# Sujit-O/pykg2vec

Hardware: AMD Instinct MI355X
Metric: scored triples/sec (train) + test-triples ranked/sec, FB15k TransE d=100 (higher is better)
Workload: dtype f32

## Files before the change

pykg2vec_amd/csrc/kge_eval.hip:

```cpp
#include "kge_internal.h"
#include <stdlib.h>
#include <string.h>

namespace kge {

#ifndef KGE_GEMM_CHUNK
#define KGE_GEMM_CHUNK 64
#endif
constexpr int kGemmChunk = KGE_GEMM_CHUNK;
constexpr int KC = 8;
constexpr int QT_PLAIN = 16;
constexpr int QT_XF = 8;

enum Form { F_L1 = 0, F_L2 = 1, F_SQM = 2, F_NEGDOT = 3 };
enum XForm { X_NONE = 0, X_TRANSH = 1, X_TRANSD = 2 };
enum Post { P_NONE = 0, P_SCALE = 1, P_CLAMP = 2, P_SIGMOID = 3 };

struct EvalPlan {
    int64_t nq;
    int only;
    int64_t E, n, tables, table_stride;
    int K, Kpad, QV, form, xform, post;
    int64_t ntiles;
    float* cand; float* aux; float* qvec; float* qscale; float* st; int32_t* fcount; int32_t* rcount; int32_t* tcount;
    float* qT;
    size_t bytes;
};

static int sweep_K(const kge_model_desc* m) {
    switch (m->model) {
        case KGE_COMPLEX: case KGE_ROTATE: case KGE_ANALOGY: return 2 * m->dim;
        case KGE_CP: case KGE_SIMPLE: case KGE_SIMPLE_IGNR: return 2 * m->dim;
        case KGE_QUATE: return 4 * m->dim;
        case KGE_TRANSR: return m->rel_dim;
        case KGE_HEAD_1N_INTERNAL: return m->dim + (m->tables[1] ? 1 : 0);
        default: return m->dim;
    }
}

static bool make_plan(const kge_model_desc* m, int64_t n, void* ws, EvalPlan* p, int64_t tables = 1) {
    p->E = m->tot_entity; p->n = n; p->nq = 2 * n; p->only = 2; p->tables = tables;
    const bool per_group_tables = tables > 1 || m->model == KGE_TRANSR;
    p->K = sweep_K(m);
    p->Kpad = (p->K + KC - 1) / KC * KC;
    p->xform = per_group_tables ? X_NONE : m->model == KGE_TRANSH ? X_TRANSH : m->model == KGE_TRANSD ? X_TRANSD : X_NONE;
    p->QV = p->xform == X_NONE ? 1 : 2;
    switch (m->model) {
        case KGE_TRANSE: case KGE_TRANSH: case KGE_TRANSD: case KGE_TRANSM: case KGE_TRANSR:
            p->form = (m->flags & KGE_FLAG_L1) ? F_L1 : F_L2; break;
        case KGE_ROTATE: p->form = F_SQM; break;
        case KGE_DISTMULT: case KGE_COMPLEX: case KGE_ANALOGY: case KGE_RESCAL:
        case KGE_CP: case KGE_SIMPLE: case KGE_SIMPLE_IGNR: case KGE_QUATE: case KGE_HEAD_1N_INTERNAL: case KGE_DOT_INTERNAL: p->form = F_NEGDOT; break;
        default: return false;
    }
    p->post = m->model == KGE_TRANSM ? P_SCALE : (m->model == KGE_SIMPLE || m->model == KGE_SIMPLE_IGNR) ? P_CLAMP
              : (m->model == KGE_HEAD_1N_INTERNAL || (m->model == KGE_DOT_INTERNAL && (m->flags & kDotSigmoid))) ? P_SIGMOID : P_NONE;
    p->ntiles = (p->E + 63) / 64;
    const bool dot_form = (p->form == F_NEGDOT || p->form == F_SQM) && p->xform == X_NONE;
    if (dot_form) p->Kpad = (p->K + 15) / 16 * 16;
    size_t off = 0;
    char* base = (char*)ws;
    auto take = [&](size_t bytes) { char* q = base ? base + off : nullptr; off += align256(bytes); return q; };
    p->table_stride = p->ntiles * p->Kpad * 64;
    p->cand = (float*)take(((size_t)tables * p->table_stride + (dot_form ? (size_t)p->Kpad * 64 : 0)) * sizeof(float));
    p->aux = (float*)take((size_t)p->ntiles * 64 * sizeof(float));
    p->qvec = (float*)take((size_t)2 * n * p->QV * p->Kpad * sizeof(float));
    p->qscale = (float*)take((size_t)2 * n * sizeof(float));
    p->st = (float*)take((size_t)2 * n * sizeof(float));
    p->fcount = (int32_t*)take((size_t)2 * n * sizeof(int32_t));
    p->rcount = (int32_t*)take((size_t)4 * n * sizeof(int32_t));
    p->tcount = p->rcount ? p->rcount + 2 * n : nullptr;
    p->qT = nullptr;
    if ((p->form == F_NEGDOT || p->form == F_SQM) && p->xform == X_NONE)
        p->qT = (float*)take((size_t)((2 * n + 127) / 128) * p->Kpad * 128 * sizeof(float));
    p->bytes = off;
    return true;
}

size_t eval_workspace_bytes(const kge_model_desc* m, int64_t n, int64_t tables) {
    if (WsBytesFn* own = model_ops(m->model)->eval_ws) return own(m, n);
    EvalPlan p;
    if (!make_plan(m, n, nullptr, &p, tables)) return 0;
    return p.bytes;
}

// ... 357 lines not shown
        for (int k = lane; k < dc; k += TPT) {
            qt[base + k] = hr[k] * rr[k] - hi[k] * ri[k];
            qt[base + dc + k] = hi[k] * rr[k] + hr[k] * ri[k];
            qh[base + k] = tr[k] * rr[k] + ti[k] * ri[k];
            qh[base + dc + k] = ti[k] * rr[k] - tr[k] * ri[k];
        }
        if constexpr (M == KGE_ANALOGY) {
            const float* eh = m.tab[0] + h * d; const float* er = m.tab[1] + r * d; const float* et = m.tab[0] + t * d;
            for (int k = lane; k < d; k += TPT) { qt[k] = eh[k] * er[k]; qh[k] = er[k] * et[k]; }
        }
    } else if constexpr (M == KGE_ROTATE) {
        const float* hr = m.tab[0] + h * d; const float* hi = m.tab[1] + h * d; const float* rl = m.tab[2] + r * d;
        const float* tr = m.tab[0] + t * d; const float* ti = m.tab[1] + t * d;
        for (int k = lane; k < d; k += TPT) {
            float sn, cs;
            sincosf(rl[k] / m.phase_div, &sn, &cs);
            qt[k] = hr[k] * cs - hi[k] * sn;
            qt[d + k] = hr[k] * sn + hi[k] * cs;
            qh[k] = tr[k] * cs + ti[k] * sn;
            qh[d + k] = ti[k] * cs - tr[k] * sn;
        }
    } else if constexpr (M == KGE_CP) {
        const float* sh = m.tab[0] + h * d; const float* er = m.tab[1] + r * d; const float* ot = m.tab[2] + t * d;
        for (int k = lane; k < d; k += TPT) {
            qt[k] = 0.f; qt[d + k] = sh[k] * er[k];
            qh[k] = er[k] * ot[k]; qh[d + k] = 0.f;
        }
    } else if constexpr (M == KGE_SIMPLE || M == KGE_SIMPLE_IGNR) {
        const float w2 = (M == KGE_SIMPLE) ? 0.5f : 1.0f;
        const float* hh = m.tab[0] + h * d; const float* ht = m.tab[0] + t * d;
        const float* th = m.tab[1] + h * d; const float* tt = m.tab[1] + t * d;
        const float* r1 = m.tab[2] + r * d; const float* r2 = m.tab[3] + r * d;
        for (int k = lane; k < d; k += TPT) {
            qt[k] = hh[k] * r1[k];
            qt[d + k] = w2 * (r2[k] * th[k]);
            qh[k] = w2 * (ht[k] * r2[k]);
            qh[d + k] = r1[k] * tt[k];
        }
    } else if constexpr (M == KGE_QUATE) {
        const float* H[4]; const float* T[4]; const float* Rq[4];
        for (int c = 0; c < 4; ++c) { H[c] = m.tab[c] + h * d; T[c] = m.tab[c] + t * d; Rq[c] = m.tab[4 + c] + r * d; }
        for (int k = lane; k < d; k += TPT) {
            const float rs = Rq[0][k], rx = Rq[1][k], ry = Rq[2][k], rz = Rq[3][k];
            const float den = sqrtf(rs * rs + rx * rx + ry * ry + rz * rz);
            const float inv = den > 0.f ? 1.0f / den : 0.f;
            const float ps = rs * inv, px = rx * inv, py = ry * inv, pz = rz * inv;
            const float hs = H[0][k], hx = H[1][k], hy = H[2][k], hz = H[3][k];
            const float ts = T[0][k], tx = T[1][k], ty = T[2][k], tz = T[3][k];
            qt[k] = hs * ps - hx * px - hy * py - hz * pz;
            qt[d + k] = hs * px + ps * hx + hy * pz - py * hz;
            qt[2 * d + k] = hs * py + ps * hy + hz * px - pz * hx;
            qt[3 * d + k] = hs * pz + ps * hz + hx * py - px * hy;
            qh[k] = ps * ts + px * tx + py * ty + pz * tz;
            qh[d + k] = -px * ts + ps * tx - pz * ty + py * tz;
            qh[2 * d + k] = -py * ts + pz * tx + ps * ty - px * tz;
            qh[3 * d + k] = -pz * ts - py * tx + px * ty + ps * tz;
        }
    } else if constexpr (M == KGE_RESCAL) {
        const float* eh = m.tab[0] + h * d; const float* et = m.tab[0] + t * d;
        const float* Mr = m.tab[1] + r * (int64_t)d * d;
        for (int j = lane; j < d; j += TPT) {
            float a = 0.f, b = 0.f;
            int i2 = 0;
            for (; i2 + KC <= d; i2 += KC) {
                float m1[KC], m2[KC], hv[KC], tv[KC];
#pragma unroll
                for (int u = 0; u < KC; ++u) {
                    m1[u] = Mr[(int64_t)(i2 + u) * d + j]; m2[u] = Mr[(int64_t)j * d + i2 + u];
                    hv[u] = eh[i2 + u]; tv[u] = et[i2 + u];
                }
#pragma unroll
                for (int u = 0; u < KC; ++u) { a = fmaf(hv[u], m1[u], a); b = fmaf(m2[u], tv[u], b); }
            }
            for (; i2 < d; ++i2) {
                a = fmaf(eh[i2], Mr[(int64_t)i2 * d + j], a);
                b = fmaf(Mr[(int64_t)j * d + i2], et[i2], b);
            }
            qt[j] = a; qh[j] = b;
        }
    }
}

__device__ __forceinline__ float add_abs(float acc, float d) { return acc + fabsf(d); }

__device__ __forceinline__ float fma_sq(float acc, float d) {
    float r;
    asm("v_fma_f32 %0, %1, %1, %2" : "=v"(r) : "v"(d), "v"(acc));
    return r;
}

template <int FORM>
__device__ __forceinline__ float pair_step(float acc, float c, float q) {
    if constexpr (FORM == F_L1) return add_abs(acc, c - q);
    else if constexpr (FORM == F_NEGDOT) return fmaf(c, q, acc);
    else { const float dlt = c - q; return fma_sq(acc, dlt); }
}
template <int FORM>
__device__ __forceinline__ float pair_finish(float acc, float margin) {
    if constexpr (FORM == F_L1) return acc;
    else if constexpr (FORM == F_L2) return sqrtf(acc);
    else if constexpr (FORM == F_SQM) return -(margin - acc);
    else return -acc;
}

template <int POST>
__device__ __forceinline__ float pair_post(float s, float scale) {
    if constexpr (POST == P_SCALE) return scale * s;
    else if constexpr (POST == P_CLAMP) return fminf(fmaxf(s, -20.f), 20.f);
    else if constexpr (POST == P_SIGMOID) return -(1.0f / (1.0f + expf(s)));
    else return s;
}

__device__ __forceinline__ float sqm_from_dot(float dot, float qn, float cn) { return fmaf(-2.0f, dot, qn + cn); }

template <int FORM, int XFORM, int POST>
__device__ __forceinline__ float pair_score_lane(const float* __restrict__ cand, const float* __restrict__ aux,
                                                 const float* __restrict__ q, int64_t e, int Kpad, float margin,
                                                 float scale) {
    const float* c = cand + ((e >> 6) * Kpad) * 64 + (e & 63);
    float acc = 0.f;
    if constexpr (XFORM == X_NONE && FORM != F_L1) {
        float a0 = 0.f, a1 = 0.f;
        for (int k0 = 0; k0 < Kpad; k0 += KC) {
            float cv[KC], qv[KC];
#pragma unroll
            for (int j = 0; j < KC; ++j) { cv[j] = c[(int64_t)(k0 + j) * 64]; qv[j] = q[k0 + j]; }
#pragma unroll
            for (int j = 0; j < KC; j += 2) {
                if constexpr (FORM == F_NEGDOT) {
                    a0 = fmaf(cv[j], qv[j], a0);
                    a1 = fmaf(cv[j + 1], qv[j + 1], a1);
                } else {
                    const float d0 = cv[j] - qv[j], d1 = cv[j + 1] - qv[j + 1];
                    a0 = fmaf(d0, d0, a0);
                    a1 = fmaf(d1, d1, a1);
                }
            }
        }
        acc = a0 + a1;
    } else if constexpr (XFORM == X_NONE) {
        constexpr int KL = 32;
        int k0 = 0;
        for (; k0 + KL <= Kpad; k0 += KL) {
            float cv[KL], qv[KL];
#pragma unroll
            for (int j = 0; j < KL; ++j) { cv[j] = c[(int64_t)(k0 + j) * 64]; qv[j] = q[k0 + j]; }
#pragma unroll
            for (int j = 0; j < KL; ++j) acc = pair_step<FORM>(acc, cv[j], qv[j]);
        }
        for (; k0 < Kpad; k0 += KC) {
            float cv[KC], qv[KC];
#pragma unroll
            for (int j = 0; j < KC; ++j) { cv[j] = c[(int64_t)(k0 + j) * 64]; qv[j] = q[k0 + j]; }
#pragma unroll
            for (int j = 0; j < KC; ++j) acc = pair_step<FORM>(acc, cv[j], qv[j]);
        }
    } else {
        const float* w = q + Kpad;
        float p;
        if constexpr (XFORM == X_TRANSH) {
            p = 0.f;
            for (int k0 = 0; k0 < Kpad; k0 += KC) {
                float cv[KC], wv[KC];
#pragma unroll
                for (int j = 0; j < KC; ++j) { cv[j] = c[(int64_t)(k0 + j) * 64]; wv[j] = w[k0 + j]; }
#pragma unroll
// ... 113 lines not shown
                    const int kk = k0 + (t & (ch - 1));
                    int ee = lc_u >= 6 ? __builtin_amdgcn_readlane(e, (64 * u) >> lc_u) : __shfl(e, (t >> lc_u) & 63, 64);
                    asm volatile("" : "+v"(ee));
                    const float* src = prep_addr(a, ee, kk);
                    if (t < total && src) v[u] = *src;
                }
            }
#pragma unroll
            for (int u = 0; u < 4; ++u) {
                const int kk = 64 * u + lane;
                qv[u] = (kk < ch && k0 + kk < Kpad) ? q[k0 + kk] : 0.f;
            }
        };
        fetch(0);
        for (int k0 = 0; k0 < Kpad; k0 += ch) {
#pragma unroll
            for (int u = 0; u < 16; ++u) {
                const int t = 64 * u + lane;
                if (64 * u < total_u && t < total) sc[(t >> lc) * pitch + (t & (ch - 1))] = v[u];
            }
#pragma unroll
            for (int u = 0; u < 4; ++u) {
                const int kk = 64 * u + lane;
                if (kk < ch) sq[kk] = qv[u];
            }
            if (k0 + ch < Kpad) fetch(k0 + ch);
            __builtin_amdgcn_wave_barrier();
            __builtin_amdgcn_s_waitcnt(0xC07F);
            if (lane < pg) {
                const float* cr = sc + lane * pitch;
                const int nk = min(ch, Kpad - k0);
                int kk = 0;
                for (; kk + 16 <= nk; kk += 16) {
                    float4 c4[4], q4[4];
#pragma unroll
                    for (int u = 0; u < 4; ++u) {
                        c4[u] = *reinterpret_cast<const float4*>(cr + kk + 4 * u);
                        q4[u] = *reinterpret_cast<const float4*>(sq + kk + 4 * u);
                    }
#pragma unroll
                    for (int u = 0; u < 4; ++u) {
                        acc = fmaf(c4[u].x, q4[u].x, acc); acc = fmaf(c4[u].y, q4[u].y, acc);
                        acc = fmaf(c4[u].z, q4[u].z, acc); acc = fmaf(c4[u].w, q4[u].w, acc);
                    }
                    if (kGemmChunk && ((k0 + kk + 16) % (kGemmChunk ? kGemmChunk : 1)) == 0) { tot += acc; acc = 0.f; }
                }
                for (; kk < nk; kk += 8) {
                    const float4 c0 = *reinterpret_cast<const float4*>(cr + kk), c1 = *reinterpret_cast<const float4*>(cr + kk + 4);
                    const float4 q0 = *reinterpret_cast<const float4*>(sq + kk), q1 = *reinterpret_cast<const float4*>(sq + kk + 4);
                    acc = fmaf(c0.x, q0.x, acc); acc = fmaf(c0.y, q0.y, acc); acc = fmaf(c0.z, q0.z, acc); acc = fmaf(c0.w, q0.w, acc);
                    acc = fmaf(c1.x, q1.x, acc); acc = fmaf(c1.y, q1.y, acc); acc = fmaf(c1.z, q1.z, acc); acc = fmaf(c1.w, q1.w, acc);
                    if (kGemmChunk && ((k0 + kk + 8) % (kGemmChunk ? kGemmChunk : 1)) == 0) { tot += acc; acc = 0.f; }
                }
            }
            __builtin_amdgcn_wave_barrier();
        }
        if (kGemmChunk) acc = tot + acc;
        if constexpr (FORM == F_SQM) acc = sqm_from_dot(acc, qn, lane < pg ? aux[e] : 0.f);
        const float sco = pair_post<POST>(pair_finish<FORM>(acc, margin), 1.0f);
        if (base == 0) s_true = __shfl(sco, 0, 64);
        if (lane < pg && idx > 0 && e != truth) cnt += (sco < s_true) ? 1 : 0;
        base += pg;
    }
    cnt = (int)wave_sum((float)cnt);
    if (lane == 0) { st[qi] = s_true; fcount[qi] = cnt; }
}

typedef float f32x2 __attribute__((ext_vector_type(2)));

template <int FORM>
__device__ __forceinline__ void pair_step2(float& acc, f32x2 c, f32x2 q) {
    if constexpr (FORM == F_NEGDOT) {
        acc = fmaf(c.x, q.x, acc);
        acc = fmaf(c.y, q.y, acc);
    } else if constexpr (FORM == F_L1) {
        acc = add_abs(acc, c.x - q.x);
        acc = add_abs(acc, c.y - q.y);
    } else {
        const f32x2 d = c - q;
        acc = fma_sq(acc, d.x); acc = fma_sq(acc, d.y);
    }
}

template <int QT, int NS, class F>
__device__ __forceinline__ void for_query_chunks(const float* const (&qrow)[QT], const int (&off)[NS], F body) {
    float nx[NS][KC];
#pragma unroll
    for (int s = 0; s < NS; ++s)
#pragma unroll
        for (int j = 0; j < KC; ++j) nx[s][j] = qrow[0][off[s] + j];
#pragma unroll
    for (int q = 0; q < QT; ++q) {
        float cur[NS][KC];
#pragma unroll
        for (int s = 0; s < NS; ++s)
#pragma unroll
            for (int j = 0; j < KC; ++j) cur[s][j] = nx[s][j];
#pragma unroll
        for (int s = 0; s < NS; ++s) asm volatile("" ::"s"(cur[s][0]), "s"(cur[s][KC - 1]));
        if (q + 1 < QT) {
#pragma unroll
            for (int s = 0; s < NS; ++s)
#pragma unroll
                for (int j = 0; j < KC; ++j) nx[s][j] = qrow[q + 1][off[s] + j];
        }
        __builtin_amdgcn_sched_barrier(0);
        body(q, cur);
        __builtin_amdgcn_sched_barrier(0);
    }
}

template <int FORM, int XFORM, int QT, bool WRITE, int POST>
__global__ __launch_bounds__(256) void k_eval_sweep(const float* __restrict__ cand, const float* __restrict__ aux,
                                                    const float* __restrict__ qvec, const float* __restrict__ qscale,
                                                    const float* __restrict__ st,
                                                    int64_t nq, int64_t E, int64_t ntiles, int Kpad, int QV, float margin,
                                                    int S, int qblocks, int32_t* __restrict__ rcount,
                                                    int32_t* __restrict__ tcount, float* __restrict__ scores_out,
                                                    const int32_t* __restrict__ qdesc, int64_t table_stride) {
    const int lane = threadIdx.x & 63;
    const int wave = threadIdx.x >> 6;
    const int slot = blockIdx.x & 255;
    const int mm = blockIdx.x >> 8;
    const int ts = mm % S;
    const int qb = (mm / S) * 256 + slot;
    if (qb >= qblocks) return;
    int64_t q0 = (int64_t)qb * QT;
    if (qdesc) {
        cand += qdesc[4 * qb] * table_stride;
        q0 = qdesc[4 * qb + 1];
        nq = q0 + qdesc[4 * qb + 2];
    }
    const int64_t qstride = (int64_t)QV * Kpad;
    const float* qrow[QT];
    float sthr[QT];
    float qsc[QT];
    int cnt[QT];
    int tie[QT];
#pragma unroll
    for (int q = 0; q < QT; ++q) {
        const int64_t qi = (q0 + q < nq) ? q0 + q : nq - 1;
        qrow[q] = qvec + qi * qstride;
        sthr[q] = WRITE ? 0.f : st[qi];
        qsc[q] = POST == P_SCALE ? qscale[qi] : 1.0f;
        cnt[q] = 0;
        tie[q] = 0;
    }
    if constexpr (XFORM == X_NONE) {
        for (int64_t tile = ((int64_t)ts * 4 + wave) * 2; tile < ntiles; tile += (int64_t)S * 8) {
            const bool has_b = tile + 1 < ntiles;
            const float* ca = cand + (tile * Kpad) * 64 + lane;
            const float* cb = has_b ? ca + (int64_t)Kpad * 64 : ca;
            float acca[QT], accb[QT];
            f32x2 pa[QT], pb[QT];
#pragma unroll
            for (int q = 0; q < QT; ++q) { acca[q] = 0.f; accb[q] = 0.f; pa[q] = f32x2{0.f, 0.f}; pb[q] = f32x2{0.f, 0.f}; }
            for (int k0 = 0; k0 < Kpad; k0 += KC) {
                f32x2 va[KC / 2], vb[KC / 2];
#pragma unroll
                for (int j = 0; j < KC / 2; ++j) {
                    va[j].x = ca[(int64_t)(k0 + 2 * j) * 64]; va[j].y = ca[(int64_t)(k0 + 2 * j + 1) * 64];
                    vb[j].x = cb[(int64_t)(k0 + 2 * j) * 64]; vb[j].y = cb[(int64_t)(k0 + 2 * j + 1) * 64];
                }
                const int off1[1] = {k0};
                for_query_chunks<QT, 1>(qrow, off1, [&](int q, const float (&qv)[1][KC]) {
#pragma unroll
                    for (int j = 0; j < KC / 2; ++j) {
                        f32x2 qq;
                        qq.x = qv[0][2 * j];
                        qq.y = qv[0][2 * j + 1];
                        if constexpr (FORM == F_NEGDOT) {
                            pa[q] = __builtin_elementwise_fma(va[j], qq, pa[q]);
                            pb[q] = __builtin_elementwise_fma(vb[j], qq, pb[q]);
                        } else if constexpr (FORM == F_L2 || FORM == F_SQM) {
                            const f32x2 da = va[j] - qq, db = vb[j] - qq;
                            pa[q] = __builtin_elementwise_fma(da, da, pa[q]);
                            pb[q] = __builtin_elementwise_fma(db, db, pb[q]);
                        } else {
                            pair_step2<FORM>(acca[q], va[j], qq);
                            pair_step2<FORM>(accb[q], vb[j], qq);
                        }
                    }
                });
            }
            if constexpr (FORM != F_L1) {
#pragma unroll
                for (int q = 0; q < QT; ++q) { acca[q] = pa[q].x + pa[q].y; accb[q] = pb[q].x + pb[q].y; }
            }
            const int64_t ea = tile * 64 + lane, eb = ea + 64;
            const bool valid_a = ea < E, valid_b = has_b && eb < E;
#pragma unroll
            for (int q = 0; q < QT; ++q) {
                const float sa = pair_post<POST>(pair_finish<FORM>(acca[q], margin), qsc[q]);
                const float sb = pair_post<POST>(pair_finish<FORM>(accb[q], margin), qsc[q]);
                if constexpr (WRITE) {
                    if (q0 + q < nq) {
                        if (valid_a) scores_out[(q0 + q) * E + ea] = sa;
                        if (valid_b) scores_out[(q0 + q) * E + eb] = sb;
                    }
                } else {
                    cnt[q] += __popcll(__ballot(valid_a && sa < sthr[q])) + __popcll(__ballot(valid_b && sb < sthr[q]));
                    tie[q] += __popcll(__ballot(valid_a && sa == sthr[q])) + __popcll(__ballot(valid_b && sb == sthr[q]));
                }
            }
        }
    } else {
    for (int64_t tile = (int64_t)ts * 4 + wave; tile < ntiles; tile += (int64_t)S * 4) {
        const float* c = cand + (tile * Kpad) * 64 + lane;
        float acc[QT];
#pragma unroll
        for (int q = 0; q < QT; ++q) acc[q] = 0.f;
        {
            float p[QT], inv[QT];
            if constexpr (XFORM == X_TRANSH) {
#pragma unroll
                for (int q = 0; q < QT; ++q) p[q] = 0.f;
                for (int k0 = 0; k0 < Kpad; k0 += KC) {
                    float cv[KC];
#pragma unroll
                    for (int j = 0; j < KC; ++j) cv[j] = c[(int64_t)(k0 + j) * 64];
                    const int off1[1] = {Kpad + k0};
                    for_query_chunks<QT, 1>(qrow, off1, [&](int q, const float (&qv)[1][KC]) {
#pragma unroll
                        for (int j = 0; j < KC; ++j) p[q] = fmaf(cv[j], qv[0][j], p[q]);
                    });
                }
#pragma unroll
                for (int q = 0; q < QT; ++q) p[q] = -p[q];
            } else {
                const float a_e = aux[tile * 64 + lane];
#pragma unroll
                for (int q = 0; q < QT; ++q) p[q] = a_e;
            }
#pragma unroll
            for (int q = 0; q < QT; ++q) inv[q] = 0.f;
            for (int k0 = 0; k0 < Kpad; k0 += KC) {
                float cv[KC];
#pragma unroll
                for (int j = 0; j < KC; ++j) cv[j] = c[(int64_t)(k0 + j) * 64];
                const int off1[1] = {Kpad + k0};
                for_query_chunks<QT, 1>(qrow, off1, [&](int q, const float (&qv)[1][KC]) {
#pragma unroll
                    for (int j = 0; j < KC; ++j) {
                        const float v = fmaf(p[q], qv[0][j], cv[j]);
                        inv[q] = fmaf(v, v, inv[q]);
                    }
                });
            }
#pragma unroll
            for (int q = 0; q < QT; ++q) inv[q] = 1.0f / fmaxf(sqrtf(inv[q]), kEpsNormalize);
            for (int k0 = 0; k0 < Kpad; k0 += KC) {
                float cv[KC];
#pragma unroll
                for (int j = 0; j < KC; ++j) cv[j] = c[(int64_t)(k0 + j) * 64];
                const int off2[2] = {Kpad + k0, k0};
                for_query_chunks<QT, 2>(qrow, off2, [&](int q, const float (&qv)[2][KC]) {
#pragma unroll
                    for (int j = 0; j < KC; ++j) {
                        const float v = fmaf(p[q], qv[0][j], cv[j]) * inv[q];
                        acc[q] = pair_step<FORM>(acc[q], v, qv[1][j]);
                    }
                });
            }
        }
        const int64_t e = tile * 64 + lane;
        const bool valid = e < E;
#pragma unroll
        for (int q = 0; q < QT; ++q) {
            const float s = pair_post<POST>(pair_finish<FORM>(acc[q], margin), qsc[q]);
            if constexpr (WRITE) {
                if (valid && q0 + q < nq) scores_out[(q0 + q) * E + e] = s;
            } else {
                cnt[q] += __popcll(__ballot(valid && s < sthr[q]));
                tie[q] += __popcll(__ballot(valid && s == sthr[q]));
            }
        }
    }
    }
    if constexpr (!WRITE) {
        if (lane == 0) {
#pragma unroll
            for (int q = 0; q < QT; ++q) {
                if (q0 + q < nq && cnt[q] != 0) atomicAdd(rcount + q0 + q, cnt[q]);
                if (tcount && q0 + q < nq && tie[q] != 0) atomicAdd(tcount + q0 + q, tie[q]);
            }
        }
    }
}

typedef float f32x16 __attribute__((ext_vector_type(16)));
constexpr int GT = 128;
#ifndef KGE_GEMM_KS
#define KGE_GEMM_KS 16
#endif
constexpr int GKS = KGE_GEMM_KS;
constexpr int GNJ = GKS / 8;
static_assert(kGemmChunk % GKS == 0, "the running total is folded at K slab boundaries");
#if defined(KGE_GEMM_32X32) && KGE_GEMM_CHUNK
#error "the 32x32x2 experiment form of k_eval_gemm keeps the single chain: build it with -DKGE_GEMM_CHUNK=0"
#endif
#ifdef KGE_GEMM_32X32
constexpr int GLD = GT + 4;
#else
constexpr int GLD = GT + 16;
#endif

__global__ __launch_bounds__(256) void k_eval_qt(const float* __restrict__ qvec, int64_t nq, int Kpad, float* __restrict__ qT) {
    __shared__ float s_t[64][65];
    const int64_t q0 = (int64_t)blockIdx.x * 64;
    const int k0 = blockIdx.y * 64;
    const int tx = threadIdx.x & 63, ty = threadIdx.x >> 6;
    for (int r = ty; r < 64; r += 4) {
        const int64_t q = q0 + r;
        s_t[r][tx] = (q < nq && k0 + tx < Kpad) ? qvec[q * Kpad + k0 + tx] : 0.f;
    }
    __syncthreads();
    for (int r = ty; r < 64; r += 4) {
        const int k = k0 + r;
        const int64_t q = q0 + tx;
        if (k < Kpad) qT[((q / GT) * Kpad + k) * GT + (q % GT)] = s_t[tx][r];
    }
}

__global__ __launch_bounds__(256) void k_eval_qnorm(const float* __restrict__ qvec, int64_t nq, int Kpad, float* __restrict__ qn) {
    const int lane = threadIdx.x & 63;
    const int64_t q = (int64_t)blockIdx.x * 4 + (threadIdx.x >> 6);
    if (q >= nq) return;
    float n2 = 0.f;
    for (int k = lane; k < Kpad; k += 64) { const float v = qvec[q * Kpad + k]; n2 = fmaf(v, v, n2); }
    n2 = wave_sum(n2);
    if (lane == 0) qn[q] = n2;
}

struct GemmSplit { int xcd, a, S, m; };
static GemmSplit gemm_split(int qtiles, int64_t ctiles, int slots_per_xcd, unsigned* grid, int S_flat) {
    GemmSplit g{0, 0, 0, 0};
    const int sw = switch_value("EVAL_GEMM_XCD");
    if (sw == 0) { *grid = (unsigned)(qtiles * S_flat); return g; }
    const int a = qtiles / 8, r = qtiles % 8;
// ... 336 lines not shown
    for (int s = 0; s < 4; ++s) { a->seg[s] = nullptr; a->seg_dim[s] = 0; }
    a->seg[0] = m->tables[0]; a->seg_dim[0] = m->dim;
    switch (m->model) {
        case KGE_TRANSE: case KGE_TRANSM: a->normalize = 1; break;
        case KGE_CP:
            a->nseg = 2; a->seg[1] = m->tables[2]; a->seg_dim[1] = m->dim; break;
        case KGE_SIMPLE: case KGE_SIMPLE_IGNR:
            a->nseg = 2; a->seg[0] = m->tables[1]; a->seg[1] = m->tables[0]; a->seg_dim[1] = m->dim; break;
        case KGE_QUATE:
            a->nseg = 4;
            for (int q = 1; q < 4; ++q) { a->seg[q] = m->tables[q]; a->seg_dim[q] = m->dim; }
            break;
        case KGE_TRANSD: a->dot_tab = m->tables[2]; break;
        case KGE_COMPLEX: case KGE_ROTATE:
            a->nseg = 2; a->seg[1] = m->tables[1]; a->seg_dim[1] = m->dim; break;
        case KGE_ANALOGY:
            a->nseg = 3; a->seg[1] = m->tables[2]; a->seg_dim[1] = m->dim / 2;
            a->seg[2] = m->tables[3]; a->seg_dim[2] = m->dim / 2; break;
        case KGE_HEAD_1N_INTERNAL:
            if (m->tables[1]) { a->nseg = 2; a->seg[1] = m->tables[1]; a->seg_dim[1] = 1; }
            break;
        default: break;
    }
}

static bool use_gemm_sweep(const EvalPlan& p, int64_t nq) {
    const int force = switch_value("EVAL_GEMM");
    if (force >= 0) return force == 1;
    return nq >= 512 && p.Kpad >= 32;
}

template <int FORM, int XFORM, int POST = P_NONE>
static void launch_tf_and_sweep(const EvalPlan& p, const kge_model_desc* m, const int64_t* triples,
                                const int64_t* tail_off, const int32_t* tail_ids, const int64_t* head_off,
                                const int32_t* head_ids, float* scores_out, hipStream_t s,
                                const int32_t* group_of_triple = nullptr, const int32_t* qdesc = nullptr,
                                int64_t n_qblocks = 0) {
    constexpr int QT = XFORM == X_NONE ? QT_PLAIN : QT_XF;
    const int64_t nq = p.nq;
    const int qblocks = qdesc ? (int)n_qblocks : (int)((nq + QT - 1) / QT);
    const int64_t tiles_per_wave_pass = XFORM == X_NONE ? 2 : 1;
    const int64_t max_split = (p.ntiles + 4 * tiles_per_wave_pass - 1) / (4 * tiles_per_wave_pass);
    const int64_t qgroups = (qblocks + 255) / 256;
    int64_t S = (48 + qgroups - 1) / qgroups;
    if (S > max_split) S = max_split;
    if (S < 1) S = 1;
    const unsigned grid = (unsigned)(qgroups * 256 * S);
    if constexpr ((FORM == F_NEGDOT || FORM == F_SQM) && XFORM == X_NONE && POST != P_SCALE) {
        if (qdesc == nullptr && p.qT != nullptr && p.Kpad % GKS == 0 && use_gemm_sweep(p, nq)) {
            constexpr bool SQM = FORM == F_SQM;
            const int qtiles = (int)((nq + GT - 1) / GT);
            const int64_t ctiles = (p.ntiles + 1) / 2;
            int64_t S2 = ((KGE_GEMM_OCC) * 256) / qtiles;
            if (S2 > ctiles) S2 = ctiles;
            if (S2 < 1) S2 = 1;
            unsigned ggrid = 0;
            const GemmSplit gs = gemm_split(qtiles, ctiles, (KGE_GEMM_OCC) * 32, &ggrid, (int)S2);
            hipLaunchKernelGGL(k_eval_qt, dim3((unsigned)(qtiles * 2), (unsigned)((p.Kpad + 63) / 64)), dim3(256), 0, s, p.qvec, nq,
                               p.Kpad, p.qT);
            if (SQM)
                hipLaunchKernelGGL(k_eval_qnorm, dim3((unsigned)((nq + 3) / 4)), dim3(256), 0, s, p.qvec, nq, p.Kpad, p.qscale);
            if (scores_out == nullptr) {
                PrepArgs pa;
                fill_prep(m, p, &pa);
                hipLaunchKernelGGL((k_eval_target_filter_chain<FORM, POST>), dim3((unsigned)((nq + 3) / 4)), dim3(256), 0, s, pa, p.aux,
                                   p.qvec, p.qscale, triples, p.n, p.Kpad, m->margin, tail_off, tail_ids, head_off, head_ids, p.st,
                                   p.fcount, p.only);
                hipLaunchKernelGGL((k_eval_gemm<false, POST, SQM>), dim3(ggrid), dim3(256), 0, s, p.cand, p.qT, p.st,
                                   nq, p.E, p.ntiles, p.Kpad, qtiles, (int)S2, gs, p.rcount, p.tcount, nullptr, p.qscale, p.aux, m->margin);
            } else {
                hipLaunchKernelGGL((k_eval_gemm<true, POST, SQM>), dim3(ggrid), dim3(256), 0, s, p.cand, p.qT, p.st,
                                   nq, p.E, p.ntiles, p.Kpad, qtiles, (int)S2, gs, p.rcount, nullptr, scores_out, p.qscale, p.aux, m->margin);
            }
            return;
        }
    }
    if (scores_out == nullptr)
        hipLaunchKernelGGL((k_eval_target_filter<FORM, XFORM, POST>), dim3((unsigned)((nq + 3) / 4)), dim3(256), 0, s, p.cand,
                           p.aux, p.qvec, p.qscale, triples, p.n, p.Kpad, p.QV, m->margin, tail_off, tail_ids, head_off, head_ids,
                           p.st, p.fcount, group_of_triple, p.table_stride, p.only);
    if (scores_out == nullptr) {
        hipLaunchKernelGGL((k_eval_sweep<FORM, XFORM, QT, false, POST>), dim3(grid), dim3(256), 0, s, p.cand, p.aux, p.qvec,
                           p.qscale, p.st, nq, p.E, p.ntiles, p.Kpad, p.QV, m->margin, (int)S, qblocks, p.rcount, p.tcount, nullptr,
                           qdesc, p.table_stride);
    } else {
        hipLaunchKernelGGL((k_eval_sweep<FORM, XFORM, QT, true, POST>), dim3(grid), dim3(256), 0, s, p.cand, p.aux, p.qvec,
                           p.qscale, p.st, nq, p.E, p.ntiles, p.Kpad, p.QV, m->margin, (int)S, qblocks, p.rcount, nullptr, scores_out,
                           qdesc, p.table_stride);
    }
}

static int run_pipeline(const kge_model_desc* m, const int64_t* triples, int64_t n, const int64_t* tail_off,
                        const int32_t* tail_ids, const int64_t* head_off, const int32_t* head_ids, void* ws,
                        size_t ws_bytes, int32_t* ranks, int32_t* ties, float* scores_out, hipStream_t s, int side) {
    EvalPlan p;
    if (!make_plan(m, n, ws, &p)) { set_error("kge_eval: model %d has no sweep form", m->model); return -1; }
    if (side != 2) {
        if ((side != 0 && side != 1) || m->model == KGE_TRANSR) {
            set_error("kge_eval: one-sided sweeps take side 0 = tail or 1 = head (TransR projects per call: use both sides)");
            return -1;
        }
        p.nq = n;
        p.only = side;
    }
    if (ws == nullptr || ws_bytes < p.bytes) {
        set_error("kge_eval: workspace too small (%zu < %zu)", ws_bytes, p.bytes);
        return -1;
    }
    if (n <= 0) return 0;
    if (m->model == KGE_TRANSR) {
        int rc = launch_transr_eval_prepare(m, triples, n, nullptr, 1, p.Kpad, p.ntiles, p.cand, p.qvec, p.qscale, s);
        if (rc) return rc;
    } else {
    PrepArgs pa;
    fill_prep(m, p, &pa);
    pa.want_n2 = (p.form == F_SQM && p.xform == X_NONE && p.qT != nullptr && use_gemm_sweep(p, p.nq)) ? 1 : 0;
    bool vec = !pa.normalize && !pa.dot_tab;
    for (int sg = 0; sg < pa.nseg; ++sg) vec = vec && pa.seg_dim[sg] % 4 == 0 && (uintptr_t)pa.seg[sg] % 16 == 0;
    if (vec) {
        const int64_t nchunks = (p.Kpad + 127) / 128;
        int64_t nky = min(nchunks, (2048 + p.ntiles - 1) / p.ntiles);
        if (pa.want_n2 && nky > 1) {
            const int64_t cap = (int64_t)((2 * n + 127) / 128) * p.Kpad * 128 / (p.ntiles * 64);
            if (cap < nky) nky = cap;
        }
        if (nky < 1) nky = 1;
        pa.kper = (int)((nchunks + nky - 1) / nky * 128);
        nky = (p.Kpad + pa.kper - 1) / pa.kper;
        float* part = (pa.want_n2 && nky > 1) ? p.qT : nullptr;
        hipLaunchKernelGGL(k_eval_prepare4, dim3((unsigned)p.ntiles, (unsigned)nky), dim3(256), 0, s, pa, p.cand, p.aux, part);
        if (part)
            hipLaunchKernelGGL(k_eval_cnorm_parts, dim3((unsigned)((p.ntiles * 64 + 255) / 256)), dim3(256), 0, s, part, (int)nky,
                               p.ntiles * 64, p.aux);
    } else {
    int ksplit = 1;
    if (!pa.normalize && !pa.dot_tab) {
        ksplit = (int)min((int64_t)((p.Kpad + 63) / 64), (4096 + p.ntiles - 1) / p.ntiles);
        if (ksplit < 1) ksplit = 1;
    }
    pa.kper = ((p.Kpad + ksplit - 1) / ksplit + 63) / 64 * 64;
    ksplit = (p.Kpad + pa.kper - 1) / pa.kper;
    hipLaunchKernelGGL(k_eval_prepare, dim3((unsigned)p.ntiles, (unsigned)ksplit), dim3(256), 0, s, pa, p.cand, p.aux);
    if (ksplit > 1 && pa.want_n2) {
        hipLaunchKernelGGL(k_eval_cnorm, dim3((unsigned)(p.ntiles * 16)), dim3(256), 0, s, pa, p.aux);
    }
    }
    const DeviceModel dm = to_device_model(m);
    const unsigned qb = (unsigned)((n + 3) / 4);
#define KGE_Q(MID) case MID: hipLaunchKernelGGL((k_eval_queries<MID>), dim3((MID == KGE_TRANSE || MID == KGE_TRANSH || MID == KGE_TRANSD || MID == KGE_TRANSM) ? qb : (unsigned)n), dim3(256), 0, s, dm, triples, n, p.K, p.Kpad, p.QV, p.qvec, p.qscale, side); break;
    switch (m->model) {
        KGE_Q(KGE_TRANSE) KGE_Q(KGE_TRANSH) KGE_Q(KGE_TRANSD) KGE_Q(KGE_ROTATE) KGE_Q(KGE_DISTMULT)
        KGE_Q(KGE_COMPLEX) KGE_Q(KGE_ANALOGY) KGE_Q(KGE_RESCAL)
        KGE_Q(KGE_TRANSM) KGE_Q(KGE_CP) KGE_Q(KGE_SIMPLE) KGE_Q(KGE_SIMPLE_IGNR) KGE_Q(KGE_QUATE) KGE_Q(KGE_HEAD_1N_INTERNAL) KGE_Q(KGE_DOT_INTERNAL)
        default: set_error("kge_eval: unsupported model %d", m->model); return -1;
    }
#undef KGE_Q
    }
    if (scores_out == nullptr) (void)hipMemsetAsync(p.rcount, 0, (size_t)4 * n * sizeof(int32_t), s);
#define KGE_S(F, X) launch_tf_and_sweep<F, X>(p, m, triples, tail_off, tail_ids, head_off, head_ids, scores_out, s)
    if (p.post == P_SCALE) {
        if (p.form == F_L1) launch_tf_and_sweep<F_L1, X_NONE, P_SCALE>(p, m, triples, tail_off, tail_ids, head_off, head_ids, scores_out, s);
        else launch_tf_and_sweep<F_L2, X_NONE, P_SCALE>(p, m, triples, tail_off, tail_ids, head_off, head_ids, scores_out, s);
    } else if (p.post == P_CLAMP) {
        launch_tf_and_sweep<F_NEGDOT, X_NONE, P_CLAMP>(p, m, triples, tail_off, tail_ids, head_off, head_ids, scores_out, s);
    } else if (p.post == P_SIGMOID) {
        launch_tf_and_sweep<F_NEGDOT, X_NONE, P_SIGMOID>(p, m, triples, tail_off, tail_ids, head_off, head_ids, scores_out, s);
    } else if (p.xform == X_NONE) {
        switch (p.form) {
            case F_L1: KGE_S(F_L1, X_NONE); break;
            case F_L2: KGE_S(F_L2, X_NONE); break;
            case F_SQM: KGE_S(F_SQM, X_NONE); break;
// ... 132 lines not shown
```

Measured before the change: 2.543 billion.

## Trim padded K tail and keep query rows in scalar registers for L1 sweep

For the L1 form, the sweep now stops the full KC-wide loop before the padded tail when the remainder is at most half a chunk. It then runs a half-width chunk instead of processing padding zeros, so with d=100 it skips four padded dimensions per candidate. Query row addressing moves to a base-plus-stride struct with a uniform clamp so row pointers stay scalar, and several asm hints pin uniform values to SGPRs. Rank counting uses direct wave-wide fcmp masks ANDed with precomputed validity ballots. The cost is more template complexity and inline-asm register constraints that could upset scheduling.

After: 2.543 billion. Within noise of the previous version (-0.0%).

```diff
diff --git a/pykg2vec_amd/csrc/kge_eval.hip b/pykg2vec_amd/csrc/kge_eval.hip
--- a/pykg2vec_amd/csrc/kge_eval.hip
+++ b/pykg2vec_amd/csrc/kge_eval.hip
@@ -1,6 +1,7 @@
 #include "kge_internal.h"
 #include <stdlib.h>
 #include <string.h>
+#include <type_traits>
 
 namespace kge {
 
@@ -524,6 +525,9 @@
 }
 
 __device__ __forceinline__ float add_abs(float acc, float d) { return acc + fabsf(d); }
+
+__device__ __forceinline__ uint64_t lanes_lt(float a, float b) { return __builtin_amdgcn_fcmpf(a, b, 4); }
+__device__ __forceinline__ uint64_t lanes_eq(float a, float b) { return __builtin_amdgcn_fcmpf(a, b, 1); }
 
 __device__ __forceinline__ float fma_sq(float acc, float d) {
     float r;
@@ -803,27 +807,34 @@
     }
 }
 
-template <int QT, int NS, class F>
-__device__ __forceinline__ void for_query_chunks(const float* const (&qrow)[QT], const int (&off)[NS], F body) {
-    float nx[NS][KC];
+struct BlockRows {
+    const float* base; unsigned stride; int last;
+    __device__ __forceinline__ const float* operator[](int q) const {
+        return (const float*)((const char*)base + (unsigned)min(q, last) * stride);
+    }
+};
+
+template <int QT, int NS, int KN = KC, class R, class F>
+__device__ __forceinline__ void for_query_chunks(const R& qrow, const int (&off)[NS], F body) {
+    float nx[NS][KN];
 #pragma unroll
     for (int s = 0; s < NS; ++s)
 #pragma unroll
-        for (int j = 0; j < KC; ++j) nx[s][j] = qrow[0][off[s] + j];
+        for (int j = 0; j < KN; ++j) nx[s][j] = qrow[0][off[s] + j];
 #pragma unroll
     for (int q = 0; q < QT; ++q) {
-        float cur[NS][KC];
+        float cur[NS][KN];
 #pragma unroll
         for (int s = 0; s < NS; ++s)
 #pragma unroll
-            for (int j = 0; j < KC; ++j) cur[s][j] = nx[s][j];
-#pragma unroll
-        for (int s = 0; s < NS; ++s) asm volatile("" ::"s"(cur[s][0]), "s"(cur[s][KC - 1]));
+            for (int j = 0; j < KN; ++j) cur[s][j] = nx[s][j];
+#pragma unroll
+        for (int s = 0; s < NS; ++s) asm volatile("" ::"s"(cur[s][0]), "s"(cur[s][KN - 1]));
         if (q + 1 < QT) {
 #pragma unroll
             for (int s = 0; s < NS; ++s)
 #pragma unroll
-                for (int j = 0; j < KC; ++j) nx[s][j] = qrow[q + 1][off[s] + j];
+                for (int j = 0; j < KN; ++j) nx[s][j] = qrow[q + 1][off[s] + j];
         }
         __builtin_amdgcn_sched_barrier(0);
         body(q, cur);
@@ -838,7 +849,7 @@
                                                     int64_t nq, int64_t E, int64_t ntiles, int Kpad, int QV, float margin,
                                                     int S, int qblocks, int32_t* __restrict__ rcount,
                                                     int32_t* __restrict__ tcount, float* __restrict__ scores_out,
-                                                    const int32_t* __restrict__ qdesc, int64_t table_stride) {
+                                                    const int32_t* __restrict__ qdesc, int64_t table_stride, int K) {
     const int lane = threadIdx.x & 63;
     const int wave = threadIdx.x >> 6;
     const int slot = blockIdx.x & 255;
@@ -853,7 +864,9 @@
         nq = q0 + qdesc[4 * qb + 2];
     }
     const int64_t qstride = (int64_t)QV * Kpad;
-    const float* qrow[QT];
+    const float* qrow_p[QT];
+    const BlockRows qrow_b = {qvec + min(q0, nq - 1) * qstride, (unsigned)qstride * 4u,
+                              __builtin_amdgcn_readfirstlane((int)max((int64_t)0, min((int64_t)(QT - 1), nq - 1 - q0)))};
     float sthr[QT];
     float qsc[QT];
     int cnt[QT];
@@ -861,32 +874,45 @@
 #pragma unroll
     for (int q = 0; q < QT; ++q) {
         const int64_t qi = (q0 + q < nq) ? q0 + q : nq - 1;
-        qrow[q] = qvec + qi * qstride;
+        qrow_p[q] = qvec + qi * qstride;
         sthr[q] = WRITE ? 0.f : st[qi];
         qsc[q] = POST == P_SCALE ? qscale[qi] : 1.0f;
         cnt[q] = 0;
         tie[q] = 0;
     }
     if constexpr (XFORM == X_NONE) {
-        for (int64_t tile = ((int64_t)ts * 4 + wave) * 2; tile < ntiles; tile += (int64_t)S * 8) {
+        const int krem = K & (KC - 1);
+        const int kfull = FORM == F_L1 && krem != 0 && krem <= KC / 2 ? K - krem : Kpad;
+        const int wave_u = FORM == F_L1 ? __builtin_amdgcn_readfirstlane(wave) : wave;
+        for (int64_t tile = ((int64_t)ts * 4 + wave_u) * 2; tile < ntiles; tile += (int64_t)S * 8) {
             const bool has_b = tile + 1 < ntiles;
-            const float* ca = cand + (tile * Kpad) * 64 + lane;
-            const float* cb = has_b ? ca + (int64_t)Kpad * 64 : ca;
+            const float* ta = cand + (tile * Kpad) * 64;
+            const float* tb = has_b ? ta + (int64_t)Kpad * 64 : ta;
+            const float* ca = ta + lane;
+            const float* cb = tb + lane;
             float acca[QT], accb[QT];
             f32x2 pa[QT], pb[QT];
 #pragma unroll
-            for (int q = 0; q < QT; ++q) { acca[q] = 0.f; accb[q] = 0.f; pa[q] = f32x2{0.f, 0.f}; pb[q] = f32x2{0.f, 0.f}; }
-            for (int k0 = 0; k0 < Kpad; k0 += KC) {
-                f32x2 va[KC / 2], vb[KC / 2];
-#pragma unroll
-                for (int j = 0; j < KC / 2; ++j) {
+            for (int q = 0; q < QT; ++q) {
+                if constexpr (FORM == F_L1) {
+                    asm volatile("v_mov_b32 %0, 0\n\tv_mov_b32 %1, 0" : "=v"(acca[q]), "=v"(accb[q]));
+                } else {
+                    acca[q] = 0.f; accb[q] = 0.f;
+                }
+                pa[q] = f32x2{0.f, 0.f}; pb[q] = f32x2{0.f, 0.f};
+            }
+            auto chunk = [&](auto kn, int k0) __attribute__((always_inline)) {
+                constexpr int KN = decltype(kn)::value;
+                f32x2 va[KN / 2], vb[KN / 2];
+#pragma unroll
+                for (int j = 0; j < KN / 2; ++j) {
                     va[j].x = ca[(int64_t)(k0 + 2 * j) * 64]; va[j].y = ca[(int64_t)(k0 + 2 * j + 1) * 64];
                     vb[j].x = cb[(int64_t)(k0 + 2 * j) * 64]; vb[j].y = cb[(int64_t)(k0 + 2 * j + 1) * 64];
                 }
                 const int off1[1] = {k0};
-                for_query_chunks<QT, 1>(qrow, off1, [&](int q, const float (&qv)[1][KC]) {
-#pragma unroll
-                    for (int j = 0; j < KC / 2; ++j) {
+                auto body = [&](int q, const float (&qv)[1][KN]) {
+#pragma unroll
+                    for (int j = 0; j < KN / 2; ++j) {
                         f32x2 qq;
                         qq.x = qv[0][2 * j];
                         qq.y = qv[0][2 * j + 1];
@@ -902,7 +928,18 @@
                             pair_step2<FORM>(accb[q], vb[j], qq);
                         }
                     }
-                });
+                };
+                if constexpr (FORM == F_L1) {
+                    BlockRows rows = qrow_b;
+                    asm volatile("" : "+s"(rows.last));
+                    for_query_chunks<QT, 1, KN>(rows, off1, body);
+                } else {
+                    for_query_chunks<QT, 1, KN>(qrow_p, off1, body);
+                }
+            };
+            for (int k0 = 0; k0 < kfull; k0 += KC) chunk(std::integral_constant<int, KC>{}, k0);
+            if constexpr (FORM == F_L1) {
+                if (kfull < K) chunk(std::integral_constant<int, KC / 2>{}, kfull);
             }
             if constexpr (FORM != F_L1) {
 #pragma unroll
@@ -910,6 +947,7 @@
             }
             const int64_t ea = tile * 64 + lane, eb = ea + 64;
             const bool valid_a = ea < E, valid_b = has_b && eb < E;
+            const uint64_t ma = __builtin_amdgcn_ballot_w64(valid_a), mb = __builtin_amdgcn_ballot_w64(valid_b);
 #pragma unroll
             for (int q = 0; q < QT; ++q) {
                 const float sa = pair_post<POST>(pair_finish<FORM>(acca[q], margin), qsc[q]);
@@ -920,10 +958,14 @@
                         if (valid_b) scores_out[(q0 + q) * E + eb] = sb;
                     }
                 } else {
-                    cnt[q] += __popcll(__ballot(valid_a && sa < sthr[q])) + __popcll(__ballot(valid_b && sb < sthr[q]));
-                    tie[q] += __popcll(__ballot(valid_a && sa == sthr[q])) + __popcll(__ballot(valid_b && sb == sthr[q]));
+                    cnt[q] += __popcll(lanes_lt(sa, sthr[q]) & ma) + __popcll(lanes_lt(sb, sthr[q]) & mb);
+                    tie[q] += __popcll(lanes_eq(sa, sthr[q]) & ma) + __popcll(lanes_eq(sb, sthr[q]) & mb);
                 }
             }
+        }
+        if constexpr (!WRITE && FORM == F_L1) {
+#pragma unroll
+            for (int q = 0; q < QT; ++q) asm volatile("" : "+s"(cnt[q]), "+s"(tie[q]));
         }
     } else {
     for (int64_t tile = (int64_t)ts * 4 + wave; tile < ntiles; tile += (int64_t)S * 4) {
@@ -941,7 +983,7 @@
 #pragma unroll
                     for (int j = 0; j < KC; ++j) cv[j] = c[(int64_t)(k0 + j) * 64];
                     const int off1[1] = {Kpad + k0};
-                    for_query_chunks<QT, 1>(qrow, off1, [&](int q, const float (&qv)[1][KC]) {
+                    for_query_chunks<QT, 1>(qrow_p, off1, [&](int q, const float (&qv)[1][KC]) {
 #pragma unroll
                         for (int j = 0; j < KC; ++j) p[q] = fmaf(cv[j], qv[0][j], p[q]);
                     });
@@ -960,7 +1002,7 @@
 #pragma unroll
                 for (int j = 0; j < KC; ++j) cv[j] = c[(int64_t)(k0 + j) * 64];
                 const int off1[1] = {Kpad + k0};
-                for_query_chunks<QT, 1>(qrow, off1, [&](int q, const float (&qv)[1][KC]) {
+                for_query_chunks<QT, 1>(qrow_p, off1, [&](int q, const float (&qv)[1][KC]) {
 #pragma unroll
                     for (int j = 0; j < KC; ++j) {
                         const float v = fmaf(p[q], qv[0][j], cv[j]);
@@ -975,7 +1017,7 @@
 #pragma unroll
                 for (int j = 0; j < KC; ++j) cv[j] = c[(int64_t)(k0 + j) * 64];
                 const int off2[2] = {Kpad + k0, k0};
-                for_query_chunks<QT, 2>(qrow, off2, [&](int q, const float (&qv)[2][KC]) {
+                for_query_chunks<QT, 2>(qrow_p, off2, [&](int q, const float (&qv)[2][KC]) {
 #pragma unroll
                     for (int j = 0; j < KC; ++j) {
                         const float v = fmaf(p[q], qv[0][j], cv[j]) * inv[q];
@@ -1478,11 +1520,11 @@
     if (scores_out == nullptr) {
         hipLaunchKernelGGL((k_eval_sweep<FORM, XFORM, QT, false, POST>), dim3(grid), dim3(256), 0, s, p.cand, p.aux, p.qvec,
                            p.qscale, p.st, nq, p.E, p.ntiles, p.Kpad, p.QV, m->margin, (int)S, qblocks, p.rcount, p.tcount, nullptr,
-                           qdesc, p.table_stride);
+                           qdesc, p.table_stride, p.K);
     } else {
         hipLaunchKernelGGL((k_eval_sweep<FORM, XFORM, QT, true, POST>), dim3(grid), dim3(256), 0, s, p.cand, p.aux, p.qvec,
                            p.qscale, p.st, nq, p.E, p.ntiles, p.Kpad, p.QV, m->margin, (int)S, qblocks, p.rcount, nullptr, scores_out,
-                           qdesc, p.table_stride);
+                           qdesc, p.table_stride, p.K);
     }
 }
 
```
